# klemens-floege/oneprot

Measured on AMD Instinct MI355X. Metric: protein-pairs/sec/node (seq+struct-token, L=512, ESM-2-150M), higher is better.
Workload: dtype bf16; 1 GPU; cfg-2: seq<->struct_token sub-step, facebook/esm2_t30_150M_UR50D / facebook/esm2_t30_150M_UR50D, L=512, 256 pairs/GPU per modality, global batch 256, output_dim 1024, CLIP local_loss+gather_with_grad, L1 0.01, Adam 1e-3, clip 1.0, sequence encoder frozen (reference default), random-init weights; global_batch=256, seq_len=512, parallelism=dp1, frozen_sequence_encoder=True

## Files before the change

include/oneprot_hip.h:

```cpp
#ifndef ONEPROT_HIP_H
#define ONEPROT_HIP_H
#include <stddef.h>
#include <stdint.h>
#ifdef __cplusplus
extern "C" {
#endif

int oneprot_abi_version(void);

int oneprot_esm_embed_fwd(const int64_t* ids, const float* table, float* x, float* row_scale, int B, int L, int d, int vocab,
                          int pad_id, int mask_id, int token_dropout, void* stream);
size_t oneprot_esm_embed_bwd_workspace(int T, int d, int vocab);
int oneprot_esm_embed_bwd(const int64_t* ids, const float* dx, const float* row_scale, float* dtable, void* workspace, int B, int L, int d,
                          int vocab, int pad_id, int mask_id, int token_dropout, int accumulate, void* stream);
int oneprot_bert_embed_fwd(const int64_t* ids, const float* word, const float* pos, const float* type0, const float* gamma, const float* beta,
                           float* x_f32, void* x_bf16, int B, int L, int d, int vocab, float eps, void* stream);

int oneprot_layernorm_fwd(const void* x, int x_is_bf16, const float* gamma, const float* beta, void* y_bf16, float* y_f32, float* mean,
                          float* rstd, int64_t T, int d, float eps, void* stream);
size_t oneprot_layernorm_bwd_workspace(int d);
int oneprot_layernorm_bwd(const void* dy, int dy_mode, const float* wrow, int L, const void* x, int x_is_bf16, const float* gamma,
                          const float* mean, const float* rstd, const float* add_to, float* dx, void* dx_bf16 ,
                          float* dgamma, float* dbeta, void* workspace, int64_t T, int d, int accumulate_param_grads, void* stream);
int oneprot_lnpool_fwd(const float* x, const int64_t* ids, int pad_id, const float* gamma, const float* beta, float* pooled, float* mean,
// ... 36 lines not shown
int oneprot_gemm_resid_ln8_error(const void* sched_ws);
int oneprot_gemm_resid_ln8_error_clear(void* sched_ws, void* stream);
void oneprot_gemm_resid_ln8_poll_bound(int polls);
int oneprot_gemm_bf16_nt_resid_ln8(const void* A, const void* W, int64_t M, int N, int K, int lda, int ldb, const float* bias, const float* resid,
                                   float* x_out, const float* gamma, const float* beta, float eps, void* h_bf16, float* stats, void* sched_ws,
                                   size_t sched_ws_bytes, void* stream);
void oneprot_gemm_ln_form(int form);
int oneprot_gemm_ln_form_get(void);
void oneprot_gemm_force_shape(int shape);
void oneprot_gemm_tune(int sup_m, int sup_n);
size_t oneprot_gemm_bf16_tn_workspace(int N, int K);
void oneprot_gemm_tn_variant(int v);
void oneprot_cu_reserve(int cus);
int oneprot_gemm_bf16_tn(const void* dY, const void* X, int64_t M, int N, int K, int ldy, int ldx, float* dW, float* dbias, void* workspace,
                         size_t workspace_bytes, int accumulate, void* stream);
int oneprot_sgemm(const float* A, const float* B, float* C, int M, int N, int K, int transA, int b_is_kn, float alpha, int accumulate, void* stream);

int oneprot_attn_fwd(const void* q, const void* k, const void* v, const float* key_bias, void* ctx, float* lse, int B, int H, int L, int hd,
                     void* stream);
size_t oneprot_attn_bwd_workspace(int B, int H, int L);
int oneprot_attn_bwd(const void* q, const void* k, const void* v, const float* key_bias, const void* ctx, const void* dctx, const float* lse,
                     const float* rope_cos, const float* rope_sin, float q_scale, void* dqkv, void* workspace, int B, int H, int L, int hd,
                     void* stream);
int oneprot_attn_fwd_dropout(const void* q, const void* k, const void* v, const float* key_bias, void* ctx, float* lse, int B, int H, int L, int hd,
                             float p, uint64_t seed, uint64_t stream_id, void* stream);
int oneprot_attn_bwd_dropout(const void* q, const void* k, const void* v, const float* key_bias, const void* ctx, const void* dctx, const float* lse,
                             const float* rope_cos, const float* rope_sin, float q_scale, void* dqkv, void* workspace, int B, int H, int L, int hd,
                             float p, uint64_t seed, uint64_t stream_id, void* stream);
int oneprot_attn_dropout_keep(void* keep, int B, int H, int L, float p, uint64_t seed, uint64_t stream_id, void* stream);
void oneprot_attn_force_bwd_path(int path);
// ... 215 lines not shown
```

oneprot_amd/csrc/check_resources.py:

```python
#!/usr/bin/env python3
import re
import subprocess
import sys

RULES = [
    (r"^void g8::k_gemm8<", 0),
    (r"^void k_gemm_tn8<", 0),
    (r"^void gln::k_gemm_ln", 0),
    (r"^void k_attn_fwd3<", 0),
    (r"^void k_attn_fwd3w<", 0),
    (r"^void k_attn_fwd2<", 16),
    (r"^void k_attn_bwd_fused<\(int\)32>", 0),
    (r"^void k_attn_bwd_fused64<\(int\)32>", 0),
    (r"^void k_layernorm_(fwd|bwd)", 0),
    (r"^void k_sim_", 0),
    (r"^(void )?k_msa_", 0),
    (r"^(void )?k_pronet_", 0),
    (r"^(void )?k_metrics_", 0),
    (r"^(void )?k_gbt_", 0),
]


def parse(text):
    out = {}
# ... 43 lines not shown
```

oneprot_amd/csrc/gemm_tn.hip:

```cpp
#include "common.h"
#include "../../include/oneprot_hip.h"

#define TN_MAX_SLAB_TILES 512

static __device__ __attribute__((aligned(16))) unsigned int g_zero_page[4] = {0, 0, 0, 0};

__device__ __forceinline__ int tn_f(int r) { return 2 * ((r & 3) | (((r >> 3) & 1) << 2)); }

__device__ __forceinline__ bf8_t tn_frag(const unsigned char* tile, int mb, int c0, int lane) {
  const int g = lane >> 4, i = lane & 15;
  const int r0 = mb + 8 * g + (i >> 2), r1 = r0 + 4;
  const int col = c0 + 4 * (i & 3);
  const int chunk = col >> 3, within = (col & 7) * 2;
  const unsigned char* p0 = tile + r0 * 256 + ((chunk ^ tn_f(r0)) << 4) + within;
  const unsigned char* p1 = tile + r1 * 256 + ((chunk ^ tn_f(r1)) << 4) + within;
  const s16x4 a = __builtin_amdgcn_ds_read_tr16_b64_v4i16((__attribute__((address_space(3))) s16x4*)p0);
  const s16x4 b = __builtin_amdgcn_ds_read_tr16_b64_v4i16((__attribute__((address_space(3))) s16x4*)p1);
  s16x8 o;
  o[0] = a[0]; o[1] = a[1]; o[2] = a[2]; o[3] = a[3]; o[4] = b[0]; o[5] = b[1]; o[6] = b[2]; o[7] = b[3];
  return __builtin_bit_cast(bf8_t, o);
}

template <int N> __device__ __forceinline__ void tn_wait_vmcnt() { asm volatile("s_waitcnt vmcnt(%0)" ::"n"(N) : "memory"); }

// ... 226 lines not shown
  o[0] = a[0]; o[1] = a[1]; o[2] = a[2]; o[3] = a[3]; o[4] = b[0]; o[5] = b[1]; o[6] = b[2]; o[7] = b[3];
  return __builtin_bit_cast(bf8_t, o);
}

#ifdef TN8_STAMP
static __device__ unsigned long long g_tn8_stamps[2 * 64 * 8];
extern "C" int oneprot_tn8_debug_read(unsigned long long* dst) { return hipMemcpyFromSymbol(dst, HIP_SYMBOL(g_tn8_stamps), sizeof(g_tn8_stamps)) == hipSuccess ? 0 : -2; }
#define TN8_ST(i) do { if (blockIdx.x == 0 && (wave & 3) == 0 && p < 64) { unsigned long long t_; asm volatile("s_memtime %0\n\ts_waitcnt lgkmcnt(0)" : "=s"(t_) :: "memory"); \
    if (lane == 0) g_tn8_stamps[(grp * 64 + p) * 8 + (i)] = t_; } } while (0)
#else
#define TN8_ST(i) do { } while (0)
#endif
#define TN8_RING 4

template <int YC, int XC>
__global__ void __launch_bounds__(512, 2) k_gemm_tn8(const bf16_t* __restrict__ dY, const bf16_t* __restrict__ X, int M, int N, int K, int ldy, int ldx,
                                                     float* __restrict__ slab, float* __restrict__ bias_slab, int tiles_k, int tiles_all, int S) {
  constexpr int MT = YC / 64, NT = XC / 32;
  constexpr int PY = YC * 2, PX = XC * 2;
  constexpr int UY = 32 * PY, UX = 32 * PX, UNIT = UY + UX;
  constexpr int YP = UY / 1024, NP = UNIT / 1024;
  constexpr int IPW = (NP + 7) / 8;
  constexpr int NBY = PY == 640 ? 1 : 2, NBX = PX == 640 ? 2 : 4;
  static_assert(MT * NT == 40 && NP == 36 && IPW == 5, "tile");
  extern __shared__ __attribute__((aligned(16))) unsigned char smem[];
  const int per_xcd = gridDim.x >> 3;
  const int xcd = blockIdx.x & 7, seq = blockIdx.x >> 3;
  const int w = xcd * per_xcd + seq;
  if (w >= tiles_all * S) return;
  const int split = w / tiles_all, tile = w - split * tiles_all;
  const int tn = tile / tiles_k, tk = tile - tn * tiles_k;
  const int n0 = tn * YC, k0 = tk * XC;
  const int tid = threadIdx.x, lane = tid & 63;
  const int wave = __builtin_amdgcn_readfirstlane(tid >> 6);
  const int grp = wave >> 2;
  const int wn = wave >> 1, wk = wave & 1;
  const int units = M >> 5, ubase = units / S, urem = units - ubase * S;
  const int P = ubase + (split < urem ? 1 : 0);
  const int u0 = split * ubase + (split < urem ? split : urem);
  const unsigned lds0 = (unsigned)(uintptr_t)LDS_PTR(smem);

  unsigned voff[IPW]; unsigned pdst[IPW]; bool isy[IPW];
#pragma unroll
  for (int i = 0; i < IPW; ++i) {
// ... 114 lines not shown
    for (int r = 0; r < 4; ++r) {
      const int n = n0 + (4 * i + wn) * 16 + fq * 4 + r;
      if (n < N) {
#pragma unroll
        for (int j = 0; j < NT; ++j) out[(size_t)n * K + k0 + (2 * j + wk) * 16 + fr] = acc[i][j][r];
      }
    }
  if (do_bias && fr == 0) {
#pragma unroll
    for (int i = 0; i < MT; ++i)
#pragma unroll
      for (int r = 0; r < 4; ++r) {
        const int n = n0 + (4 * i + wn) * 16 + fq * 4 + r;
        if (n < N) bias_slab[(size_t)split * N + n] = accb[i][r];
      }
  }
}

static int tn8_config(int N, int K) {
  if (K % 320 == 0 && N % 256 == 0) return 1;
  if (N % 320 == 0 && K % 256 == 0) return 2;
  if (K % 320 == 0 && N >= 256 && N % 64 == 0) return 1;
  return 0;
}
static int tn8_tiles(int cfg, int N, int K) { return cfg == 1 ? ((N + 255) / 256) * (K / 320) : (N / 320) * (K / 256); }
static int g_cu_reserve = 0;
extern "C" void oneprot_cu_reserve(int cus) { g_cu_reserve = cus < 0 ? 0 : cus; }
static int tn8_cus_all() {
  static int n_cu = 0;
  if (n_cu == 0) {
// ... 92 lines not shown
    if (!c2) { if (hipFuncSetAttribute((const void*)k_gemm_tn<64, 2, 2, true>, hipFuncAttributeMaxDynamicSharedMemorySize, 2 * 2 * 64 * 256) != hipSuccess) return OP_ELAUNCH; c2 = true; }
    hipLaunchKernelGGL((k_gemm_tn<64, 2, 2, true>), dim3(8 * ((tiles * S + 7) / 8)), dim3(256), 2 * 2 * 64 * 256, s, (const bf16_t*)dY, (const bf16_t*)X, (int)M, N, K, ldy, ldx,
                       (float*)workspace, bias_slab, tiles_k, tiles, S, m_per);
  } else {
    static bool c1 = false;
    if (!c1) { if (hipFuncSetAttribute((const void*)k_gemm_tn<32, 3, 3, false>, hipFuncAttributeMaxDynamicSharedMemorySize, 3 * 2 * 32 * 256) != hipSuccess) return OP_ELAUNCH; c1 = true; }
    hipLaunchKernelGGL((k_gemm_tn<32, 3, 3, false>), dim3(8 * ((tiles * S + 7) / 8)), dim3(256), 3 * 2 * 32 * 256, s, (const bf16_t*)dY, (const bf16_t*)X, (int)M, N, K, ldy, ldx,
                       (float*)workspace, bias_slab, tiles_k, tiles, S, m_per);
  }
  const size_t n4 = ((size_t)N * K) >> 2;
  size_t blocks = (n4 + 255) / 256; if (blocks > 4096) blocks = 4096;
  const int bb = dbias ? (N + 255) / 256 : 0;
  hipLaunchKernelGGL(k_tn_reduce, dim3((unsigned)blocks + bb), dim3(256), 0, s, (const float*)workspace, dW, n4, n4, S, accumulate, (const float*)bias_slab, dbias, N, bb);
  return launch_status();
}
```

oneprot_amd/csrc/rowops.hip:

```cpp
#include "common.h"
#include "../../include/oneprot_hip.h"

#define MAXV 8
#define ROWS_PER_BLOCK 4

struct RowSeg { size_t base; int L; bool tail; bool ok; };
template <bool VAR>
__device__ __forceinline__ RowSeg row_seg(int b, int L_or_T_pad, const int* __restrict__ cu, int N) {
  if constexpr (!VAR) {
    return {(size_t)b * L_or_T_pad, L_or_T_pad, false, true};
  } else {
    const bool tail = b == N;
    const int base = cu[b], L = (tail ? L_or_T_pad : cu[b + 1]) - base;
    return {(size_t)base, L, tail, L > 0 && base >= 0 && base + L <= L_or_T_pad};
  }
}

template <bool VAR>
__global__ void __launch_bounds__(256) k_embed_fwd(const long long* __restrict__ ids, const int* __restrict__ cu, const float* __restrict__ W,
                                                   const float* __restrict__ rope_cos, const float* __restrict__ rope_sin, float* __restrict__ x,
                                                   float* __restrict__ scale_out, float* __restrict__ cos_out, float* __restrict__ sin_out, int N,
                                                   int L_or_T_pad, int d, int vocab, int half, int n_pos, int pad_id, int mask_id, int token_dropout,
                                                   int tok_per_block) {
  const int b = blockIdx.y, chunk = blockIdx.x, tid = threadIdx.x;
// ... 244 lines not shown
#pragma unroll
  for (int i = 0; i < NV; ++i) {
    dg[i] = make_float4(0, 0, 0, 0);
    db[i] = make_float4(0, 0, 0, 0);
  }
  for (int row = blockIdx.x * ROWS_PER_BLOCK + wave; row < T; row += gridDim.x * ROWS_PER_BLOCK) {
    const float mean = mean_in[row], rstd = rstd_in[row];
    float w = 1.0f;
    size_t dyrow = (size_t)row / (DY_MODE == 2 ? L : 1);
    if (DY_MODE >= 2) w = wrow[row];
    if (DY_MODE == 3) {
      int lo = 0, hi = L - 1;
      while (lo < hi) { const int mid = (lo + hi + 1) >> 1; if (cu[mid] <= row) lo = mid; else hi = mid - 1; }
      dyrow = lo;
    }
    float4 xh[NV], g[NV];
#ifndef LN_BWD_LATE_ADD
    float4 av[NV];
    if (add_to) {
#pragma unroll
      for (int i = 0; i < NV; ++i) {
        const int c = lane + 64 * i;
        if (c < nv4) av[i] = reinterpret_cast<const float4*>(add_to + (size_t)row * d)[c];
      }
    }
#endif
    float s1 = 0.f, s2 = 0.f;
#pragma unroll
    for (int i = 0; i < NV; ++i) {
      const int c = lane + 64 * i;
      if (c < nv4) {
        float4 xv;
        if (X_BF16) {
          const u32x2 p = reinterpret_cast<const u32x2*>((const bf16_t*)x + (size_t)row * d)[c];
          xv = make_float4(bflo(p.x), bfhi(p.x), bflo(p.y), bfhi(p.y));
        } else {
          xv = reinterpret_cast<const float4*>((const float*)x + (size_t)row * d)[c];
        }
        float4 dyv;
        if (DY_MODE == 0) {
          const u32x2 p = reinterpret_cast<const u32x2*>((const bf16_t*)dy + (size_t)row * d)[c];
          dyv = make_float4(bflo(p.x), bfhi(p.x), bflo(p.y), bfhi(p.y));
        } else if (DY_MODE == 1) {
          dyv = reinterpret_cast<const float4*>((const float*)dy + (size_t)row * d)[c];
        } else {
          dyv = reinterpret_cast<const float4*>((const float*)dy + dyrow * d)[c];
          dyv.x *= w; dyv.y *= w; dyv.z *= w; dyv.w *= w;
        }
        xh[i] = make_float4((xv.x - mean) * rstd, (xv.y - mean) * rstd, (xv.z - mean) * rstd, (xv.w - mean) * rstd);
        const float4 gm = reinterpret_cast<const float4*>(gamma)[c];
        g[i] = make_float4(dyv.x * gm.x, dyv.y * gm.y, dyv.z * gm.z, dyv.w * gm.w);
        s1 += (g[i].x + g[i].y) + (g[i].z + g[i].w);
        s2 += (g[i].x * xh[i].x + g[i].y * xh[i].y) + (g[i].z * xh[i].z + g[i].w * xh[i].w);
        dg[i].x += dyv.x * xh[i].x; dg[i].y += dyv.y * xh[i].y; dg[i].z += dyv.z * xh[i].z; dg[i].w += dyv.w * xh[i].w;
        db[i].x += dyv.x; db[i].y += dyv.y; db[i].z += dyv.z; db[i].w += dyv.w;
      }
    }
    const float m1 = wave_sum(s1) * inv_d, m2 = wave_sum(s2) * inv_d;
#pragma unroll
    for (int i = 0; i < NV; ++i) {
      const int c = lane + 64 * i;
      if (c < nv4) {
        float4 o;
        o.x = rstd * (g[i].x - m1 - xh[i].x * m2);
        o.y = rstd * (g[i].y - m1 - xh[i].y * m2);
        o.z = rstd * (g[i].z - m1 - xh[i].z * m2);
        o.w = rstd * (g[i].w - m1 - xh[i].w * m2);
        if (add_to) {
#ifdef LN_BWD_LATE_ADD
          const float4 a = reinterpret_cast<const float4*>(add_to + (size_t)row * d)[c];
#else
          const float4 a = av[i];
#endif
          o.x += a.x; o.y += a.y; o.z += a.z; o.w += a.w;
        }
        reinterpret_cast<float4*>(dx_out + (size_t)row * d)[c] = o;
        if (dx_bf16) { u32x2 pk; pk.x = pack2bf(o.x, o.y); pk.y = pack2bf(o.z, o.w); reinterpret_cast<u32x2*>(dx_bf16 + (size_t)row * d)[c] = pk; }
      }
    }
  }
  if (partial) {
    float* pw = s_part + (size_t)wave * 2 * d;
#pragma unroll
    for (int i = 0; i < NV; ++i) {
      const int c = lane + 64 * i;
      if (c < nv4) {
        reinterpret_cast<float4*>(pw)[c] = dg[i];
        reinterpret_cast<float4*>(pw + d)[c] = db[i];
      }
    }
    __syncthreads();
    float* pg = partial + (size_t)blockIdx.x * 2 * d;
    for (int j = threadIdx.x; j < 2 * d; j += 256)
      pg[j] = (s_part[j] + s_part[2 * d + j]) + (s_part[4 * d + j] + s_part[6 * d + j]);
  }
}

#define LN_BWD_BLOCKS 1024
extern "C" size_t oneprot_layernorm_bwd_workspace(int d) { return (size_t)LN_BWD_BLOCKS * 2 * d * sizeof(float); }

__global__ void __launch_bounds__(1024) k_ln_reduce(const float* __restrict__ partial, float* __restrict__ dgamma, float* __restrict__ dbeta, int nparts, int d, int accumulate) {
  __shared__ float s_sl[64][17];
  const int c = threadIdx.x & 15, sl = threadIdx.x >> 4;
  const int j = blockIdx.x * 16 + c;
  float s = 0.f;
  if (j < 2 * d)
    for (int p = sl; p < nparts; p += 64) s += partial[(size_t)p * 2 * d + j];
  s_sl[sl][c] = s;
  __syncthreads();
  if (sl < 4) {
    float t = 0.f;
#pragma unroll
    for (int q = 0; q < 16; ++q) t += s_sl[sl * 16 + q][c];
    s_sl[sl][c] = t;
  }
  __syncthreads();
  if (sl == 0 && j < 2 * d) {
    const float t = (s_sl[0][c] + s_sl[1][c]) + (s_sl[2][c] + s_sl[3][c]);
    float* out = j < d ? dgamma + j : dbeta + (j - d);
    *out = accumulate ? *out + t : t;
  }
}

extern "C" int oneprot_layernorm_bwd(const void* dy, int dy_mode, const float* wrow, int L, const void* x, int x_is_bf16, const float* gamma,
                                     const float* mean, const float* rstd, const float* add_to, float* dx, void* dx_bf16, float* dgamma, float* dbeta,
                                     void* workspace, int64_t T, int d, int accumulate_param_grads, void* stream) {
  if (!dy || !x || !gamma || !mean || !rstd || !dx || T <= 0 || (d & 3) || d > MAXV * 256) return OP_EINVAL;
  if (dy_mode < 0 || dy_mode > 2 || (dy_mode == 2 && (!wrow || L <= 0))) return OP_EINVAL;
  if ((dgamma || dbeta) && !(dgamma && dbeta && workspace)) return OP_EINVAL;
  int blocks = (int)((T + ROWS_PER_BLOCK - 1) / ROWS_PER_BLOCK);
  if (blocks > LN_BWD_BLOCKS) blocks = LN_BWD_BLOCKS;
  float* partial = dgamma ? (float*)workspace : nullptr;
  hipStream_t s = (hipStream_t)stream;
  const int nv = (d / 4 + 63) / 64;
  const size_t lds = partial ? (size_t)4 * 2 * d * sizeof(float) : 0;
  if (lds > 64 * 1024) return OP_EINVAL;
#define LAUNCH_LNB(M, XB, N) hipLaunchKernelGGL((k_layernorm_bwd<M, XB, N>), dim3(blocks), dim3(256), lds, s, dy, wrow, L, x, gamma, mean, rstd, add_to, dx, (bf16_t*)dx_bf16, partial, (int)T, d)
// ... 642 lines not shown
```

oneprot_amd/esm.py:

```python
import json
import os
from collections import OrderedDict

import torch
import torch.nn as nn

from . import hip
from . import layout
from .arena import ArenaModule, ModelConfig, load_weight_file, _Out
from .lora import LoraArena

KNOWN_ESM = {
    "esm2_t6_8M_UR50D": dict(num_hidden_layers=6, hidden_size=320, intermediate_size=1280),
    "esm2_t12_35M_UR50D": dict(num_hidden_layers=12, hidden_size=480, intermediate_size=1920),
    "esm2_t30_150M_UR50D": dict(num_hidden_layers=30, hidden_size=640, intermediate_size=2560),
    "esm2_t33_650M_UR50D": dict(num_hidden_layers=33, hidden_size=1280, intermediate_size=5120),
}
ESM_DEFAULTS = dict(model_type="esm", vocab_size=33, pad_token_id=1, mask_token_id=32, num_attention_heads=20, layer_norm_eps=1e-5,
                    token_dropout=True, position_embedding_type="rotary", emb_layer_norm_before=False, max_position_embeddings=1026,
                    initializer_range=0.02, hidden_dropout_prob=0.0, attention_probs_dropout_prob=0.0)


def resolve_config(model_name_or_path, defaults_by_type=None):
    path = str(model_name_or_path)
# ... 374 lines not shown
        dev = g.device
        gv = lambda name: self.view(name, gflat)
        b16 = lambda *s: torch.empty(*s, dtype=torch.bfloat16, device=dev)
        ws_ln = torch.empty(hip.query("oneprot_layernorm_bwd_workspace", d), dtype=torch.uint8, device=dev)
        lora_raw, lora_tn = self._lora_backward_setup(saved, dev)
        ws_tn = self._tn_workspace(((3 * dp, d), (f, d), (d, f), (d, dp)) + lora_tn, dev)
        ws_at = lay.attn_workspace(H, dev)
        dz = b16(T, f)
        dh = b16(T, d)
        dctx = b16(T, dp) if self._padded else dh
        dqkv = b16(T, 3 * dp)
        ready_hi = self._total
        if self._padded:
            rowmap, colmap = self._head_pad_maps()
            gw_qkv, gb_qkv, gw_o = torch.empty(3 * dp, d, device=dev), torch.empty(3 * dp, device=dev), torch.empty(d, dp, device=dev)
        bounds = saved.get("bounds")
        seg_of_top = {hi - 1: (lo, hi) for lo, hi in saved["plan"][:-1]} if bounds is not None else {}
        for i in reversed(range(self.n_layers)):
            if i in seg_of_top:
                self._recompute_segment(saved, *seg_of_top[i])
            st = saved["layers"][i]
            p = f"encoder.layer.{i}."
            self._wgrad(g16, st["u"], T, d, f, gv(p + "output.dense.weight"), gv(p + "output.dense.bias"), ws_tn)
            hip.gemm_nt(g16, self._bf16_T[(i, "w2")], T, f, d, hip.EPI_GELU_BWD, dz, aux=st["z"])
            self._wgrad(dz, st["h2"], T, f, d, gv(p + "intermediate.dense.weight"), gv(p + "intermediate.dense.bias"), ws_tn)
            hip.gemm_nt(dz, self._bf16_T[(i, "w1")], T, d, f, hip.EPI_BF16, dh)
            hip.layernorm_bwd(dh, 0, st["x_mid"], self.view(p + "LayerNorm.weight"), st["mean2"], st["rstd2"], g, gv(p + "LayerNorm.weight"), gv(p + "LayerNorm.bias"),
                              ws_ln, T, d, add_to=g, dx16=g16)
            hip.gemm_tn(g16, st["ctx"], T, d, dp, gw_o if self._padded else gv(p + "attention.output.dense.weight"), gv(p + "attention.output.dense.bias"), ws_tn)
            hip.gemm_nt(g16, self._bf16_T[(i, "o")], T, dp, d, hip.EPI_BF16, dctx)
            lay.attn_bwd(st, dctx, q_scale, dqkv, ws_at, H, hd)
            (o, n), (ob, nb) = self._qkv_spans(i)
            hip.gemm_tn(dqkv, st["h1"], T, 3 * dp, d, gw_qkv if self._padded else gflat[o:o + n], gb_qkv if self._padded else gflat[ob:ob + nb], ws_tn)
            if self._padded:
                gv(p + "attention.output.dense.weight").copy_(gw_o[:, colmap])
                gflat[o:o + n].view(3 * d, d).copy_(gw_qkv[rowmap])
                gflat[ob:ob + nb].copy_(gb_qkv[rowmap])
            hip.gemm_nt(dqkv, self._bf16_T[(i, "qkv")], T, d, 3 * dp, hip.EPI_BF16, dh)
            if lora_raw is not None:
                self._lora_branch_backward(i, st["h1"], st["lora_u"], dqkv, T, saved["lora_call"], ws_tn, lora_raw, dh16=dh)
            hip.layernorm_bwd(dh, 0, st["x_in"], self.view(p + "attention.LayerNorm.weight"), st["mean1"], st["rstd1"], g, gv(p + "attention.LayerNorm.weight"),
                              gv(p + "attention.LayerNorm.bias"), ws_ln, T, d, add_to=g, dx16=g16)
            saved["layers"][i] = st = None
            if bounds is not None:
                bounds.pop(i, None)
            if on_ready is not None and i > 0 and i % self.GRAD_CHUNK_LAYERS == 0:
                lo = self._spec[f"encoder.layer.{i}.attention.self.query.weight"][0]
                on_ready(lo, ready_hi)
                ready_hi = lo
        lay.embed_bwd(self, g, gv("embeddings.word_embeddings.weight"))
        if on_ready is not None:
            on_ready(0, ready_hi)

    @torch.no_grad()
    def forward(self, input_ids=None, attention_mask=None, **_):
        x, _ = self.run_layers(input_ids, save=False)
        return _Out(layout.of(self, input_ids).final_hidden(self, x))
# ... 15 lines not shown
```

oneprot_amd/hip.py:

```python
import ctypes
import os
import re
from ctypes import c_float, c_int, c_int64, c_size_t, c_uint64, c_void_p

import torch

_HERE = os.path.dirname(os.path.abspath(__file__))
LIB_PATH = os.environ.get("ONEPROT_HIP_LIB") or os.path.join(_HERE, "liboneprot_hip.so")

ABI_VERSION = 7
EPI_BF16, EPI_F32, EPI_BIAS_GELU, EPI_BIAS_RESID, EPI_QKV_ROPE, EPI_GELU_BWD = range(6)
LOG2E = 1.4426950408889634


class HipLibraryMissing(RuntimeError):
    pass


class HipKernelError(RuntimeError):
    pass


HEADER_PATH = os.path.join(os.path.dirname(_HERE), "include", "oneprot_hip.h")

# ... 152 lines not shown
    call("oneprot_gemm_bf16_nt", a, w, M, N, K, K if lda is None else lda, K if ldb is None else ldb, epi, bias, out0, out1, out2, aux, cos, sin, q_scale, L, H, hd)


def gemm_tn(dY, X, M, N, K, dW, dbias, ws, *, ldy=None, ldx=None, accumulate=0):
    call("oneprot_gemm_bf16_tn", dY, X, M, N, K, N if ldy is None else ldy, K if ldx is None else ldx, dW, dbias, ws, ws.numel(), accumulate)


def layernorm_fwd(x, gamma, beta, T, d, eps, *, y16=None, y32=None, mean=None, rstd=None, x_is_bf16=0):
    call("oneprot_layernorm_fwd", x, x_is_bf16, gamma, beta, y16, y32, mean, rstd, T, d, eps)


def layernorm_bwd(dy, dy_mode, x, gamma, mean, rstd, dx, dgamma, dbeta, ws, T, d, *, wrow=None, L=0, x_is_bf16=0, add_to=None, dx16=None, accumulate=0):
    call("oneprot_layernorm_bwd", dy, dy_mode, wrow, L, x, x_is_bf16, gamma, mean, rstd, add_to, dx, dx16, dgamma, dbeta, ws, T, d, accumulate)


def _workspace(query_name, like, *shape):
    nbytes = query(query_name, *shape)
    if nbytes == 0:
        raise HipKernelError(f"{query_name}{shape} returned 0: invalid size")
    return torch.empty(nbytes, dtype=torch.uint8, device=like.device)


def sort_f32(keys, *, descending=False, want_keys=False):
    n = keys.numel()
    perm = torch.empty(n, dtype=torch.int32, device=keys.device)
    out = torch.empty(n, dtype=torch.float32, device=keys.device) if want_keys else None
    ws = _workspace("oneprot_sort_workspace", keys, n)
    call("oneprot_sort_f32", keys, n, int(bool(descending)), perm, out, ws, ws.numel())
    return perm, out

# ... 168 lines not shown
```

Baseline: 1212 protein-pairs/sec/node.

## Co-schedule weight-gradient GEMM and LayerNorm backward in one kernel launch

Adds a combined kernel where the first blocks compute the split-K weight-gradient GEMM tiles and the remaining reserved CU blocks run the LayerNorm backward rows concurrently, with a prefetch ring for row loads. In the ESM backward pass the intermediate wgrad and the QKV wgrad are deferred and paired with the following LayerNorm backward, so the two memory- and compute-bound stages overlap instead of running serially. The LN row math is factored into a shared header. This reduces the CUs available to the GEMM and reorders work, which may cost GEMM throughput if the split is badly balanced.

```diff
diff --git a/include/oneprot_hip.h b/include/oneprot_hip.h
--- a/include/oneprot_hip.h
+++ b/include/oneprot_hip.h
@@ -74,6 +74,11 @@
 void oneprot_cu_reserve(int cus);
 int oneprot_gemm_bf16_tn(const void* dY, const void* X, int64_t M, int N, int K, int ldy, int ldx, float* dW, float* dbias, void* workspace,
                          size_t workspace_bytes, int accumulate, void* stream);
+int oneprot_gemm_tn_ln_bwd_eligible(int64_t M, int N, int K);
+int oneprot_gemm_tn_ln_bwd(const void* dY, const void* X, int64_t M, int N, int K, int ldy, int ldx, float* dW, float* dbias, void* workspace,
+                           size_t workspace_bytes, int accumulate, const void* dy, const float* x, const float* gamma, const float* mean, const float* rstd,
+                           const float* add_to, float* dx, void* dx_bf16, float* dgamma, float* dbeta, float* ln_partial, int accumulate_param_grads,
+                           int ln_cus, void* stream);
 int oneprot_sgemm(const float* A, const float* B, float* C, int M, int N, int K, int transA, int b_is_kn, float alpha, int accumulate, void* stream);
 
 int oneprot_attn_fwd(const void* q, const void* k, const void* v, const float* key_bias, void* ctx, float* lse, int B, int H, int L, int hd,
diff --git a/oneprot_amd/csrc/check_resources.py b/oneprot_amd/csrc/check_resources.py
--- a/oneprot_amd/csrc/check_resources.py
+++ b/oneprot_amd/csrc/check_resources.py
@@ -6,6 +6,7 @@
 RULES = [
     (r"^void g8::k_gemm8<", 0),
     (r"^void k_gemm_tn8<", 0),
+    (r"^void k_gemm_tn8_ln<", 0),
     (r"^void gln::k_gemm_ln", 0),
     (r"^void k_attn_fwd3<", 0),
     (r"^void k_attn_fwd3w<", 0),
diff --git a/oneprot_amd/csrc/gemm_tn.hip b/oneprot_amd/csrc/gemm_tn.hip
--- a/oneprot_amd/csrc/gemm_tn.hip
+++ b/oneprot_amd/csrc/gemm_tn.hip
@@ -1,4 +1,5 @@
 #include "common.h"
+#include "ln_bwd_row.h"
 #include "../../include/oneprot_hip.h"
 
 #define TN_MAX_SLAB_TILES 512
@@ -264,8 +265,8 @@
 #define TN8_RING 4
 
 template <int YC, int XC>
-__global__ void __launch_bounds__(512, 2) k_gemm_tn8(const bf16_t* __restrict__ dY, const bf16_t* __restrict__ X, int M, int N, int K, int ldy, int ldx,
-                                                     float* __restrict__ slab, float* __restrict__ bias_slab, int tiles_k, int tiles_all, int S) {
+__device__ __forceinline__ void tn8_work_item(int w, const bf16_t* __restrict__ dY, const bf16_t* __restrict__ X, int M, int N, int K, int ldy, int ldx,
+                                              float* __restrict__ slab, float* __restrict__ bias_slab, int tiles_k, int tiles_all, int S) {
   constexpr int MT = YC / 64, NT = XC / 32;
   constexpr int PY = YC * 2, PX = XC * 2;
   constexpr int UY = 32 * PY, UX = 32 * PX, UNIT = UY + UX;
@@ -274,10 +275,6 @@
   constexpr int NBY = PY == 640 ? 1 : 2, NBX = PX == 640 ? 2 : 4;
   static_assert(MT * NT == 40 && NP == 36 && IPW == 5, "tile");
   extern __shared__ __attribute__((aligned(16))) unsigned char smem[];
-  const int per_xcd = gridDim.x >> 3;
-  const int xcd = blockIdx.x & 7, seq = blockIdx.x >> 3;
-  const int w = xcd * per_xcd + seq;
-  if (w >= tiles_all * S) return;
   const int split = w / tiles_all, tile = w - split * tiles_all;
   const int tn = tile / tiles_k, tk = tile - tn * tiles_k;
   const int n0 = tn * YC, k0 = tk * XC;
@@ -422,6 +419,83 @@
         const int n = n0 + (4 * i + wn) * 16 + fq * 4 + r;
         if (n < N) bias_slab[(size_t)split * N + n] = accb[i][r];
       }
+  }
+}
+
+template <int YC, int XC>
+__global__ void __launch_bounds__(512, 2) k_gemm_tn8(const bf16_t* __restrict__ dY, const bf16_t* __restrict__ X, int M, int N, int K, int ldy, int ldx,
+                                                     float* __restrict__ slab, float* __restrict__ bias_slab, int tiles_k, int tiles_all, int S) {
+  const int per_xcd = gridDim.x >> 3;
+  const int xcd = blockIdx.x & 7, seq = blockIdx.x >> 3;
+  const int w = xcd * per_xcd + seq;
+  if (w >= tiles_all * S) return;
+  tn8_work_item<YC, XC>(w, dY, X, M, N, K, ldy, ldx, slab, bias_slab, tiles_k, tiles_all, S);
+}
+
+template <int NV>
+__global__ void __launch_bounds__(512, 2) k_gemm_tn8_ln(const bf16_t* __restrict__ dY, const bf16_t* __restrict__ X, int M, int N, int K, int ldy, int ldx,
+                                                        float* __restrict__ slab, float* __restrict__ bias_slab, int tiles_k, int tiles_all, int S, int n_tn,
+                                                        const bf16_t* __restrict__ dy, const float* __restrict__ x, const float* __restrict__ gamma,
+                                                        const float* __restrict__ mean_in, const float* __restrict__ rstd_in, const float* add_to, float* dx_out,
+                                                        bf16_t* __restrict__ dx_bf16, float* __restrict__ partial) {
+  constexpr int LN_AHEAD = NV <= 4 ? 2 : 1;
+  if ((int)blockIdx.x < n_tn) {
+    const int per_xcd = n_tn >> 3;
+    const int xcd = blockIdx.x & 7, seq = blockIdx.x >> 3;
+    const int w = xcd * per_xcd + seq;
+    if (w >= tiles_all * S) return;
+    tn8_work_item<256, 320>(w, dY, X, M, N, K, ldy, ldx, slab, bias_slab, tiles_k, tiles_all, S);
+    return;
+  }
+  extern __shared__ __attribute__((aligned(16))) unsigned char smem[];
+  float* s_part = reinterpret_cast<float*>(smem);
+  const int T = M, d = K;
+  const int lane = threadIdx.x & 63, wave = __builtin_amdgcn_readfirstlane(threadIdx.x >> 6);
+  const int rb = (int)blockIdx.x - n_tn, stride = ((int)gridDim.x - n_tn) * 8;
+  const int nv4 = d >> 2;
+  const float inv_d = 1.0f / (float)d;
+  float4 dg[NV], db[NV];
+#pragma unroll
+  for (int i = 0; i < NV; ++i) {
+    dg[i] = make_float4(0, 0, 0, 0);
+    db[i] = make_float4(0, 0, 0, 0);
+  }
+  float4 gm[NV];
+#pragma unroll
+  for (int i = 0; i < NV; ++i)
+    gm[i] = lane + 64 * i < nv4 ? reinterpret_cast<const float4*>(gamma)[lane + 64 * i] : make_float4(0, 0, 0, 0);
+  LnBwdRow<NV> ring[LN_AHEAD + 1];
+  const int row0 = rb * 8 + wave;
+  auto clamped = [&](int row, int s) { return (int)min((long long)row + (long long)s * stride, (long long)T - 1); };
+  if (row0 < T) {
+#pragma unroll
+    for (int s = 0; s < LN_AHEAD; ++s) ln_bwd_row_load(ring[s], clamped(row0, s), dy, x, mean_in, rstd_in, add_to, lane, nv4, d);
+    for (int row = row0; row < T;) {
+#pragma unroll
+      for (int s = 0; s <= LN_AHEAD; ++s) {
+        ln_bwd_row_load(ring[(s + LN_AHEAD) % (LN_AHEAD + 1)], clamped(row, LN_AHEAD), dy, x, mean_in, rstd_in, add_to, lane, nv4, d);
+        ln_bwd_row<0, NV>(LnBwdRowSrc<NV>{ring[s], gm}, row, ring[s].mean, ring[s].rstd, 1.0f, gamma, add_to != nullptr, dx_out, dx_bf16, dg, db, lane, nv4, d, inv_d);
+        row += stride;
+        if (row >= T) goto rows_done;
+      }
+    }
+  }
+rows_done:
+  if (partial) {
+    float* pw = s_part + (size_t)wave * 2 * d;
+#pragma unroll
+    for (int i = 0; i < NV; ++i) {
+      const int c = lane + 64 * i;
+      if (c < nv4) {
+        reinterpret_cast<float4*>(pw)[c] = dg[i];
+        reinterpret_cast<float4*>(pw + d)[c] = db[i];
+      }
+    }
+    __syncthreads();
+    float* pg = partial + (size_t)rb * 2 * d;
+    for (int j = threadIdx.x; j < 2 * d; j += 512)
+      pg[j] = ((s_part[j] + s_part[2 * d + j]) + (s_part[4 * d + j] + s_part[6 * d + j])) +
+              ((s_part[8 * d + j] + s_part[10 * d + j]) + (s_part[12 * d + j] + s_part[14 * d + j]));
   }
 }
 
@@ -544,3 +618,62 @@
   hipLaunchKernelGGL(k_tn_reduce, dim3((unsigned)blocks + bb), dim3(256), 0, s, (const float*)workspace, dW, n4, n4, S, accumulate, (const float*)bias_slab, dbias, N, bb);
   return launch_status();
 }
+
+static int tn8_ln_splits(int64_t M, int tiles, int reserve) {
+  int n_cu = tn8_cus_all() - reserve;
+  if (n_cu < 64) n_cu = 64;
+  int S = tn8_splits(M, tiles, n_cu, 64);
+  if (S > 0) return S;
+  S = n_cu / tiles;
+  if (S > 64) S = 64;
+  if (S > M / 256) S = (int)(M / 256);
+  return S < 1 ? 1 : S;
+}
+
+extern "C" int oneprot_gemm_tn_ln_bwd_eligible(int64_t M, int N, int K) {
+  return M > 0 && M <= 0x7fffffff && N > 0 && K > 0 && !(N & 7) && tn8_config(N, K) == 1 && M % 32 == 0 && !(K & 3) && K <= 5 * 256;
+}
+
+extern "C" int oneprot_gemm_tn_ln_bwd(const void* dY, const void* X, int64_t M, int N, int K, int ldy, int ldx, float* dW, float* dbias, void* workspace,
+                                      size_t workspace_bytes, int accumulate, const void* dy, const float* x, const float* gamma, const float* mean, const float* rstd,
+                                      const float* add_to, float* dx, void* dx_bf16, float* dgamma, float* dbeta, float* ln_partial, int accumulate_param_grads,
+                                      int ln_cus, void* stream) {
+  if (!dY || !X || !dW || !workspace || M <= 0 || N <= 0 || K <= 0 || M > 0x7fffffff) return OP_EINVAL;
+  if ((N & 7) || (ldy & 7) || (ldx & 7) || ldy < N || ldx < K) return OP_EINVAL;
+  if (((uintptr_t)dY | (uintptr_t)X | (uintptr_t)dW | (uintptr_t)workspace) & 15) return OP_EINVAL;
+  if (!dy || !x || !gamma || !mean || !rstd || !dx) return OP_EINVAL;
+  if ((dgamma || dbeta) && !(dgamma && dbeta && ln_partial)) return OP_EINVAL;
+  if (((uintptr_t)dy & 7) || (((uintptr_t)x | (uintptr_t)gamma | (uintptr_t)dx | (uintptr_t)add_to | (uintptr_t)ln_partial) & 15) || ((uintptr_t)dx_bf16 & 7)) return OP_EINVAL;
+  if (!oneprot_gemm_tn_ln_bwd_eligible(M, N, K)) return OP_EINVAL;
+  if (ln_cus < 8 || (ln_cus & 7) || ln_cus > tn8_cus_all() - 64) return OP_EINVAL;
+  if ((size_t)32 * ldy * 2 >= (1u << 31) || (size_t)32 * ldx * 2 >= (1u << 31)) return OP_EINVAL;
+  const int tiles = tn8_tiles(1, N, K);
+  const int S = tn8_ln_splits(M, tiles, ln_cus);
+  const size_t per_split = (size_t)N * K * sizeof(float) + (dbias ? (size_t)N * sizeof(float) : 0);
+  if (workspace_bytes < (size_t)S * per_split) return OP_EINVAL;
+  constexpr int LDS8 = TN8_RING * 36 * 1024;
+  static bool c8 = false;
+  if (!c8) {
+    if (hipFuncSetAttribute((const void*)k_gemm_tn8_ln<2>, hipFuncAttributeMaxDynamicSharedMemorySize, LDS8) != hipSuccess) return OP_ELAUNCH;
+    if (hipFuncSetAttribute((const void*)k_gemm_tn8_ln<3>, hipFuncAttributeMaxDynamicSharedMemorySize, LDS8) != hipSuccess) return OP_ELAUNCH;
+    if (hipFuncSetAttribute((const void*)k_gemm_tn8_ln<4>, hipFuncAttributeMaxDynamicSharedMemorySize, LDS8) != hipSuccess) return OP_ELAUNCH;
+    if (hipFuncSetAttribute((const void*)k_gemm_tn8_ln<5>, hipFuncAttributeMaxDynamicSharedMemorySize, LDS8) != hipSuccess) return OP_ELAUNCH;
+    c8 = true;
+  }
+  hipStream_t s = (hipStream_t)stream;
+  float* bias_slab = dbias ? (float*)workspace + (size_t)S * N * K : nullptr;
+  const int n_tn = 8 * ((tiles * S + 7) / 8);
+  float* partial = dgamma ? ln_partial : nullptr;
+  const int nv = (K / 4 + 63) / 64;
+#define LAUNCH_TNLN(NV) hipLaunchKernelGGL((k_gemm_tn8_ln<NV>), dim3(n_tn + ln_cus), dim3(512), LDS8, s, (const bf16_t*)dY, (const bf16_t*)X, (int)M, N, K, ldy, ldx, (float*)workspace, \
+                                           bias_slab, K / 320, tiles, S, n_tn, (const bf16_t*)dy, x, gamma, mean, rstd, add_to, dx, (bf16_t*)dx_bf16, partial)
+  if (nv <= 2) LAUNCH_TNLN(2); else if (nv == 3) LAUNCH_TNLN(3); else if (nv == 4) LAUNCH_TNLN(4); else LAUNCH_TNLN(5);
+#undef LAUNCH_TNLN
+  const size_t n4 = ((size_t)N * K) >> 2;
+  size_t blocks = (n4 + 255) / 256; if (blocks > 4096) blocks = 4096;
+  const int bb = dbias ? (N + 255) / 256 : 0;
+  hipLaunchKernelGGL(k_tn_reduce, dim3((unsigned)blocks + bb), dim3(256), 0, s, (const float*)workspace, dW, n4, n4, S, accumulate, (const float*)bias_slab, dbias, N, bb);
+  if (dgamma)
+    hipLaunchKernelGGL(k_ln_reduce, dim3((2 * K + 15) / 16), dim3(1024), 0, s, (const float*)ln_partial, dgamma, dbeta, ln_cus, K, accumulate_param_grads);
+  return launch_status();
+}
diff --git a/oneprot_amd/csrc/ln_bwd_row.h b/oneprot_amd/csrc/ln_bwd_row.h
--- /dev/null
+++ b/oneprot_amd/csrc/ln_bwd_row.h
@@ -0,0 +1,132 @@
+#pragma once
+#include "common.h"
+
+template <int DY_MODE, int X_BF16, int NV>
+struct LnBwdDirect {
+  const void* __restrict__ dy; const void* __restrict__ x; const float* add_to;
+  size_t row, dyrow; int d;
+  float4 av[NV];
+  __device__ __forceinline__ void begin(int lane, int nv4) {
+#ifndef LN_BWD_LATE_ADD
+    if (add_to) {
+#pragma unroll
+      for (int i = 0; i < NV; ++i) {
+        const int c = lane + 64 * i;
+        if (c < nv4) av[i] = reinterpret_cast<const float4*>(add_to + row * d)[c];
+      }
+    }
+#endif
+  }
+  __device__ __forceinline__ auto xraw(int i, int c) const {
+    if constexpr (X_BF16) return reinterpret_cast<const u32x2*>((const bf16_t*)x + row * d)[c];
+    else return reinterpret_cast<const float4*>((const float*)x + row * d)[c];
+  }
+  __device__ __forceinline__ auto dyraw(int i, int c) const {
+    if constexpr (DY_MODE == 0) return reinterpret_cast<const u32x2*>((const bf16_t*)dy + row * d)[c];
+    else if constexpr (DY_MODE == 1) return reinterpret_cast<const float4*>((const float*)dy + row * d)[c];
+    else return reinterpret_cast<const float4*>((const float*)dy + dyrow * d)[c];
+  }
+  __device__ __forceinline__ float4 gamma4(int i, int c, const float* __restrict__ gamma) const { return reinterpret_cast<const float4*>(gamma)[c]; }
+  __device__ __forceinline__ float4 add(int i, int c) const {
+#ifdef LN_BWD_LATE_ADD
+    return reinterpret_cast<const float4*>(add_to + row * d)[c];
+#else
+    return av[i];
+#endif
+  }
+};
+
+template <int NV>
+struct LnBwdRow {
+  float4 xv[NV]; u32x2 dyp[NV]; float4 av[NV];
+  float mean, rstd;
+};
+template <int NV>
+struct LnBwdRowSrc {
+  const LnBwdRow<NV>& r; const float4 (&gm)[NV];
+  __device__ __forceinline__ float4 xraw(int i, int) const { return r.xv[i]; }
+  __device__ __forceinline__ u32x2 dyraw(int i, int) const { return r.dyp[i]; }
+  __device__ __forceinline__ float4 gamma4(int i, int, const float*) const { return gm[i]; }
+  __device__ __forceinline__ float4 add(int i, int) const { return r.av[i]; }
+};
+template <int NV>
+__device__ __forceinline__ void ln_bwd_row_load(LnBwdRow<NV>& r, int row, const bf16_t* __restrict__ dy, const float* __restrict__ x, const float* __restrict__ mean_in,
+                                                const float* __restrict__ rstd_in, const float* add_to, int lane, int nv4, int d) {
+  r.mean = mean_in[row];
+  r.rstd = rstd_in[row];
+  const float* ap = add_to ? add_to : x;
+#pragma unroll
+  for (int i = 0; i < NV; ++i) {
+    const int c = min(lane + 64 * i, nv4 - 1);
+    r.av[i] = reinterpret_cast<const float4*>(ap + (size_t)row * d)[c];
+    r.xv[i] = reinterpret_cast<const float4*>(x + (size_t)row * d)[c];
+    r.dyp[i] = reinterpret_cast<const u32x2*>(dy + (size_t)row * d)[c];
+  }
+}
+
+__device__ __forceinline__ float4 ln_bwd_f4(const float4& v) { return v; }
+__device__ __forceinline__ float4 ln_bwd_f4(const u32x2& p) { return make_float4(bflo(p.x), bfhi(p.x), bflo(p.y), bfhi(p.y)); }
+
+template <int DY_MODE, int NV, class Src>
+__device__ __forceinline__ void ln_bwd_row(const Src& src, int row, float mean, float rstd, float w, const float* __restrict__ gamma, bool has_add, float* dx_out,
+                                           bf16_t* __restrict__ dx_bf16, float4 (&dg)[NV], float4 (&db)[NV], int lane, int nv4, int d, float inv_d) {
+  float4 xh[NV], g[NV];
+  float s1 = 0.f, s2 = 0.f;
+#pragma unroll
+  for (int i = 0; i < NV; ++i) {
+    const int c = lane + 64 * i;
+    if (c < nv4) {
+      const float4 xv = ln_bwd_f4(src.xraw(i, c));
+      float4 dyv = ln_bwd_f4(src.dyraw(i, c));
+      if (DY_MODE >= 2) { dyv.x *= w; dyv.y *= w; dyv.z *= w; dyv.w *= w; }
+      xh[i] = make_float4((xv.x - mean) * rstd, (xv.y - mean) * rstd, (xv.z - mean) * rstd, (xv.w - mean) * rstd);
+      const float4 gm = src.gamma4(i, c, gamma);
+      g[i] = make_float4(dyv.x * gm.x, dyv.y * gm.y, dyv.z * gm.z, dyv.w * gm.w);
+      s1 += (g[i].x + g[i].y) + (g[i].z + g[i].w);
+      s2 += (g[i].x * xh[i].x + g[i].y * xh[i].y) + (g[i].z * xh[i].z + g[i].w * xh[i].w);
+      dg[i].x += dyv.x * xh[i].x; dg[i].y += dyv.y * xh[i].y; dg[i].z += dyv.z * xh[i].z; dg[i].w += dyv.w * xh[i].w;
+      db[i].x += dyv.x; db[i].y += dyv.y; db[i].z += dyv.z; db[i].w += dyv.w;
+    }
+  }
+  const float m1 = wave_sum(s1) * inv_d, m2 = wave_sum(s2) * inv_d;
+#pragma unroll
+  for (int i = 0; i < NV; ++i) {
+    const int c = lane + 64 * i;
+    if (c < nv4) {
+      float4 o;
+      o.x = rstd * (g[i].x - m1 - xh[i].x * m2);
+      o.y = rstd * (g[i].y - m1 - xh[i].y * m2);
+      o.z = rstd * (g[i].z - m1 - xh[i].z * m2);
+      o.w = rstd * (g[i].w - m1 - xh[i].w * m2);
+      if (has_add) {
+        const float4 a = src.add(i, c);
+        o.x += a.x; o.y += a.y; o.z += a.z; o.w += a.w;
+      }
+      reinterpret_cast<float4*>(dx_out + (size_t)row * d)[c] = o;
+      if (dx_bf16) { u32x2 pk; pk.x = pack2bf(o.x, o.y); pk.y = pack2bf(o.z, o.w); reinterpret_cast<u32x2*>(dx_bf16 + (size_t)row * d)[c] = pk; }
+    }
+  }
+}
+
+static __global__ void __launch_bounds__(1024) k_ln_reduce(const float* __restrict__ partial, float* __restrict__ dgamma, float* __restrict__ dbeta, int nparts, int d, int accumulate) {
+  __shared__ float s_sl[64][17];
+  const int c = threadIdx.x & 15, sl = threadIdx.x >> 4;
+  const int j = blockIdx.x * 16 + c;
+  float s = 0.f;
+  if (j < 2 * d)
+    for (int p = sl; p < nparts; p += 64) s += partial[(size_t)p * 2 * d + j];
+  s_sl[sl][c] = s;
+  __syncthreads();
+  if (sl < 4) {
+    float t = 0.f;
+#pragma unroll
+    for (int q = 0; q < 16; ++q) t += s_sl[sl * 16 + q][c];
+    s_sl[sl][c] = t;
+  }
+  __syncthreads();
+  if (sl == 0 && j < 2 * d) {
+    const float t = (s_sl[0][c] + s_sl[1][c]) + (s_sl[2][c] + s_sl[3][c]);
+    float* out = j < d ? dgamma + j : dbeta + (j - d);
+    *out = accumulate ? *out + t : t;
+  }
+}
diff --git a/oneprot_amd/csrc/rowops.hip b/oneprot_amd/csrc/rowops.hip
--- a/oneprot_amd/csrc/rowops.hip
+++ b/oneprot_amd/csrc/rowops.hip
@@ -1,4 +1,5 @@
 #include "common.h"
+#include "ln_bwd_row.h"
 #include "../../include/oneprot_hip.h"
 
 #define MAXV 8
@@ -282,70 +283,9 @@
       while (lo < hi) { const int mid = (lo + hi + 1) >> 1; if (cu[mid] <= row) lo = mid; else hi = mid - 1; }
       dyrow = lo;
     }
-    float4 xh[NV], g[NV];
-#ifndef LN_BWD_LATE_ADD
-    float4 av[NV];
-    if (add_to) {
-#pragma unroll
-      for (int i = 0; i < NV; ++i) {
-        const int c = lane + 64 * i;
-        if (c < nv4) av[i] = reinterpret_cast<const float4*>(add_to + (size_t)row * d)[c];
-      }
-    }
-#endif
-    float s1 = 0.f, s2 = 0.f;
-#pragma unroll
-    for (int i = 0; i < NV; ++i) {
-      const int c = lane + 64 * i;
-      if (c < nv4) {
-        float4 xv;
-        if (X_BF16) {
-          const u32x2 p = reinterpret_cast<const u32x2*>((const bf16_t*)x + (size_t)row * d)[c];
-          xv = make_float4(bflo(p.x), bfhi(p.x), bflo(p.y), bfhi(p.y));
-        } else {
-          xv = reinterpret_cast<const float4*>((const float*)x + (size_t)row * d)[c];
-        }
-        float4 dyv;
-        if (DY_MODE == 0) {
-          const u32x2 p = reinterpret_cast<const u32x2*>((const bf16_t*)dy + (size_t)row * d)[c];
-          dyv = make_float4(bflo(p.x), bfhi(p.x), bflo(p.y), bfhi(p.y));
-        } else if (DY_MODE == 1) {
-          dyv = reinterpret_cast<const float4*>((const float*)dy + (size_t)row * d)[c];
-        } else {
-          dyv = reinterpret_cast<const float4*>((const float*)dy + dyrow * d)[c];
-          dyv.x *= w; dyv.y *= w; dyv.z *= w; dyv.w *= w;
-        }
-        xh[i] = make_float4((xv.x - mean) * rstd, (xv.y - mean) * rstd, (xv.z - mean) * rstd, (xv.w - mean) * rstd);
-        const float4 gm = reinterpret_cast<const float4*>(gamma)[c];
-        g[i] = make_float4(dyv.x * gm.x, dyv.y * gm.y, dyv.z * gm.z, dyv.w * gm.w);
-        s1 += (g[i].x + g[i].y) + (g[i].z + g[i].w);
-        s2 += (g[i].x * xh[i].x + g[i].y * xh[i].y) + (g[i].z * xh[i].z + g[i].w * xh[i].w);
-        dg[i].x += dyv.x * xh[i].x; dg[i].y += dyv.y * xh[i].y; dg[i].z += dyv.z * xh[i].z; dg[i].w += dyv.w * xh[i].w;
-        db[i].x += dyv.x; db[i].y += dyv.y; db[i].z += dyv.z; db[i].w += dyv.w;
-      }
-    }
-    const float m1 = wave_sum(s1) * inv_d, m2 = wave_sum(s2) * inv_d;
-#pragma unroll
-    for (int i = 0; i < NV; ++i) {
-      const int c = lane + 64 * i;
-      if (c < nv4) {
-        float4 o;
-        o.x = rstd * (g[i].x - m1 - xh[i].x * m2);
-        o.y = rstd * (g[i].y - m1 - xh[i].y * m2);
-        o.z = rstd * (g[i].z - m1 - xh[i].z * m2);
-        o.w = rstd * (g[i].w - m1 - xh[i].w * m2);
-        if (add_to) {
-#ifdef LN_BWD_LATE_ADD
-          const float4 a = reinterpret_cast<const float4*>(add_to + (size_t)row * d)[c];
-#else
-          const float4 a = av[i];
-#endif
-          o.x += a.x; o.y += a.y; o.z += a.z; o.w += a.w;
-        }
-        reinterpret_cast<float4*>(dx_out + (size_t)row * d)[c] = o;
-        if (dx_bf16) { u32x2 pk; pk.x = pack2bf(o.x, o.y); pk.y = pack2bf(o.z, o.w); reinterpret_cast<u32x2*>(dx_bf16 + (size_t)row * d)[c] = pk; }
-      }
-    }
+    LnBwdDirect<DY_MODE, X_BF16, NV> src{dy, x, add_to, (size_t)row, dyrow, d};
+    src.begin(lane, nv4);
+    ln_bwd_row<DY_MODE, NV>(src, row, mean, rstd, w, gamma, add_to != nullptr, dx_out, dx_bf16, dg, db, lane, nv4, d, inv_d);
   }
   if (partial) {
     float* pw = s_part + (size_t)wave * 2 * d;
@@ -366,29 +306,6 @@
 
 #define LN_BWD_BLOCKS 1024
 extern "C" size_t oneprot_layernorm_bwd_workspace(int d) { return (size_t)LN_BWD_BLOCKS * 2 * d * sizeof(float); }
-
-__global__ void __launch_bounds__(1024) k_ln_reduce(const float* __restrict__ partial, float* __restrict__ dgamma, float* __restrict__ dbeta, int nparts, int d, int accumulate) {
-  __shared__ float s_sl[64][17];
-  const int c = threadIdx.x & 15, sl = threadIdx.x >> 4;
-  const int j = blockIdx.x * 16 + c;
-  float s = 0.f;
-  if (j < 2 * d)
-    for (int p = sl; p < nparts; p += 64) s += partial[(size_t)p * 2 * d + j];
-  s_sl[sl][c] = s;
-  __syncthreads();
-  if (sl < 4) {
-    float t = 0.f;
-#pragma unroll
-    for (int q = 0; q < 16; ++q) t += s_sl[sl * 16 + q][c];
-    s_sl[sl][c] = t;
-  }
-  __syncthreads();
-  if (sl == 0 && j < 2 * d) {
-    const float t = (s_sl[0][c] + s_sl[1][c]) + (s_sl[2][c] + s_sl[3][c]);
-    float* out = j < d ? dgamma + j : dbeta + (j - d);
-    *out = accumulate ? *out + t : t;
-  }
-}
 
 extern "C" int oneprot_layernorm_bwd(const void* dy, int dy_mode, const float* wrow, int L, const void* x, int x_is_bf16, const float* gamma,
                                      const float* mean, const float* rstd, const float* add_to, float* dx, void* dx_bf16, float* dgamma, float* dbeta,
diff --git a/oneprot_amd/esm.py b/oneprot_amd/esm.py
--- a/oneprot_amd/esm.py
+++ b/oneprot_amd/esm.py
@@ -412,6 +412,8 @@
         if self._padded:
             rowmap, colmap = self._head_pad_maps()
             gw_qkv, gb_qkv, gw_o = torch.empty(3 * dp, d, device=dev), torch.empty(3 * dp, device=dev), torch.empty(d, dp, device=dev)
+        wg_ln = (hip.wgrad_ln_wanted() and not self._lora and not self._padded and hip.cu_reserve_wanted() == 0 and int(os.environ.get("WORLD_SIZE", "1")) == 1
+                 and hip.query("oneprot_gemm_tn_ln_bwd_eligible", T, f, d) == 1 and hip.query("oneprot_gemm_tn_ln_bwd_eligible", T, 3 * dp, d) == 1)
         bounds = saved.get("bounds")
         seg_of_top = {hi - 1: (lo, hi) for lo, hi in saved["plan"][:-1]} if bounds is not None else {}
         for i in reversed(range(self.n_layers)):
@@ -421,15 +423,22 @@
             p = f"encoder.layer.{i}."
             self._wgrad(g16, st["u"], T, d, f, gv(p + "output.dense.weight"), gv(p + "output.dense.bias"), ws_tn)
             hip.gemm_nt(g16, self._bf16_T[(i, "w2")], T, f, d, hip.EPI_GELU_BWD, dz, aux=st["z"])
-            self._wgrad(dz, st["h2"], T, f, d, gv(p + "intermediate.dense.weight"), gv(p + "intermediate.dense.bias"), ws_tn)
-            hip.gemm_nt(dz, self._bf16_T[(i, "w1")], T, d, f, hip.EPI_BF16, dh)
-            hip.layernorm_bwd(dh, 0, st["x_mid"], self.view(p + "LayerNorm.weight"), st["mean2"], st["rstd2"], g, gv(p + "LayerNorm.weight"), gv(p + "LayerNorm.bias"),
-                              ws_ln, T, d, add_to=g, dx16=g16)
+            if wg_ln:
+                hip.gemm_nt(dz, self._bf16_T[(i, "w1")], T, d, f, hip.EPI_BF16, dh)
+                hip.gemm_tn_ln_bwd(dz, st["h2"], T, f, d, gv(p + "intermediate.dense.weight"), gv(p + "intermediate.dense.bias"), ws_tn, dh, st["x_mid"],
+                                   self.view(p + "LayerNorm.weight"), st["mean2"], st["rstd2"], g, gv(p + "LayerNorm.weight"), gv(p + "LayerNorm.bias"), ws_ln,
+                                   hip.wgrad_ln_cus(f), add_to=g, dx16=g16)
+            else:
+                self._wgrad(dz, st["h2"], T, f, d, gv(p + "intermediate.dense.weight"), gv(p + "intermediate.dense.bias"), ws_tn)
+                hip.gemm_nt(dz, self._bf16_T[(i, "w1")], T, d, f, hip.EPI_BF16, dh)
+                hip.layernorm_bwd(dh, 0, st["x_mid"], self.view(p + "LayerNorm.weight"), st["mean2"], st["rstd2"], g, gv(p + "LayerNorm.weight"), gv(p + "LayerNorm.bias"),
+                                  ws_ln, T, d, add_to=g, dx16=g16)
             hip.gemm_tn(g16, st["ctx"], T, d, dp, gw_o if self._padded else gv(p + "attention.output.dense.weight"), gv(p + "attention.output.dense.bias"), ws_tn)
             hip.gemm_nt(g16, self._bf16_T[(i, "o")], T, dp, d, hip.EPI_BF16, dctx)
             lay.attn_bwd(st, dctx, q_scale, dqkv, ws_at, H, hd)
             (o, n), (ob, nb) = self._qkv_spans(i)
-            hip.gemm_tn(dqkv, st["h1"], T, 3 * dp, d, gw_qkv if self._padded else gflat[o:o + n], gb_qkv if self._padded else gflat[ob:ob + nb], ws_tn)
+            if not wg_ln:
+                hip.gemm_tn(dqkv, st["h1"], T, 3 * dp, d, gw_qkv if self._padded else gflat[o:o + n], gb_qkv if self._padded else gflat[ob:ob + nb], ws_tn)
             if self._padded:
                 gv(p + "attention.output.dense.weight").copy_(gw_o[:, colmap])
                 gflat[o:o + n].view(3 * d, d).copy_(gw_qkv[rowmap])
@@ -437,8 +446,13 @@
             hip.gemm_nt(dqkv, self._bf16_T[(i, "qkv")], T, d, 3 * dp, hip.EPI_BF16, dh)
             if lora_raw is not None:
                 self._lora_branch_backward(i, st["h1"], st["lora_u"], dqkv, T, saved["lora_call"], ws_tn, lora_raw, dh16=dh)
-            hip.layernorm_bwd(dh, 0, st["x_in"], self.view(p + "attention.LayerNorm.weight"), st["mean1"], st["rstd1"], g, gv(p + "attention.LayerNorm.weight"),
-                              gv(p + "attention.LayerNorm.bias"), ws_ln, T, d, add_to=g, dx16=g16)
+            if wg_ln:
+                hip.gemm_tn_ln_bwd(dqkv, st["h1"], T, 3 * dp, d, gflat[o:o + n], gflat[ob:ob + nb], ws_tn, dh, st["x_in"], self.view(p + "attention.LayerNorm.weight"),
+                                   st["mean1"], st["rstd1"], g, gv(p + "attention.LayerNorm.weight"), gv(p + "attention.LayerNorm.bias"), ws_ln,
+                                   hip.wgrad_ln_cus(3 * dp), add_to=g, dx16=g16)
+            else:
+                hip.layernorm_bwd(dh, 0, st["x_in"], self.view(p + "attention.LayerNorm.weight"), st["mean1"], st["rstd1"], g, gv(p + "attention.LayerNorm.weight"),
+                                  gv(p + "attention.LayerNorm.bias"), ws_ln, T, d, add_to=g, dx16=g16)
             saved["layers"][i] = st = None
             if bounds is not None:
                 bounds.pop(i, None)
diff --git a/oneprot_amd/hip.py b/oneprot_amd/hip.py
--- a/oneprot_amd/hip.py
+++ b/oneprot_amd/hip.py
@@ -190,6 +190,23 @@
     call("oneprot_layernorm_bwd", dy, dy_mode, wrow, L, x, x_is_bf16, gamma, mean, rstd, add_to, dx, dx16, dgamma, dbeta, ws, T, d, accumulate)
 
 
+def gemm_tn_ln_bwd(dY, X, M, N, K, dW, dbias, ws, dy, x, gamma, mean, rstd, dx, dgamma, dbeta, ws_ln, ln_cus, *, add_to=None, dx16=None):
+    call("oneprot_gemm_tn_ln_bwd", dY, X, M, N, K, N, K, dW, dbias, ws, ws.numel(), 0, dy, x, gamma, mean, rstd, add_to, dx, dx16, dgamma, dbeta, ws_ln.view(torch.float32), 0,
+         ln_cus)
+
+
+WGRAD_LN_CUS = {2560: 64, 1920: 80}
+
+
+def wgrad_ln_wanted():
+    return os.environ.get("ONEPROT_WGRAD_LN", "1") != "0"
+
+
+def wgrad_ln_cus(N):
+    v = os.environ.get("ONEPROT_WGRAD_LN_CUS")
+    return int(v) if v else WGRAD_LN_CUS.get(N, 64)
+
+
 def _workspace(query_name, like, *shape):
     nbytes = query(query_name, *shape)
     if nbytes == 0:
```

Measured after the change: 1236 protein-pairs/sec/node (median of 6 runs). 2.0% higher.
